# manycore-research/PlankAssembly

Measured on AMD Instinct MI355X. Metric: train samples/sec (fwd+bwd+all-reduce+Adam), d_model=512 seq=1024 [value: bf16 MFMA, f32 accumulate / master weights; train.f32 / train.x3: the same step in exact f32 / f32 with bf16x3 products = the parity paths], higher is better.
Workload: dtype bf16; 1 GPU; train_complete.yaml model d_model=512 H=8 dff=1024 6+6 post-norm layers, dropout 0.2, S=1024 (MAX_INPUT_LENGTH 1025), T=128, batch 16/GPU; global_batch=16, seq_len=1024, parallelism=dp1

## Files before the change

include/plank_hip.h:

```cpp
#ifndef PLANK_HIP_H
#define PLANK_HIP_H
#include <stdint.h>

#ifdef __cplusplus
extern "C" {
#endif

#define PA_F32 0
#define PA_BF16 1

#define PA_EINVAL (-1)
#define PA_EALIGN (-2)
#define PA_ESHAPE (-3)

int pa_version(void);

typedef struct {
    const void* A; const void* B; void* C;
    const float* bias;
    const void* R;
    const void* aux;
    void* ws;
    int32_t M, N, K;
    int32_t lda, ldb, ldc, ldr, ldaux;
// ... 216 lines not shown
                 float b2, float eps, int32_t step, float gscale, void* stream);
int pa_cast(void* dst, int32_t dst_dtype, const void* src, int32_t src_dtype, int64_t n, void* stream);

#define PA_GRAD_GUARD_PARTIALS 2048
typedef struct {
    float norm, coef, step_size, inv_sqrt_bc2;
    int32_t apply, applied, skipped, attempts, first_skipped_attempt;
    int32_t pad_[7];
} pa_grad_guard_ctl;
int64_t pa_grad_guard_ws_bytes(void);
int pa_grad_guard_init(void* ws, int64_t ws_bytes, int32_t step0, void* stream);
int pa_grad_guard(const float* g, int64_t n, float gscale, float max_norm, int32_t skip_nonfinite, float lr, float b1,
                  float b2, void* ws, int64_t ws_bytes, void* stream);
int pa_adam_step_guarded(float* p, const float* g, float* m, float* v, void* p_bf16, int64_t n, float b1, float b2,
                         float eps, float gscale, float clip_value, const pa_grad_guard_ctl* ctl, void* stream);
int pa_fake_collective(void* buf, int64_t bytes, int32_t blocks, int32_t passes, float min_us, void* stream);

typedef struct pa_model pa_model;
typedef struct {
    int32_t d_model, n_head, d_ff, n_enc, n_dec, vocab;
    int32_t out_dof;
    int32_t in_table_rows[5];
    float eps_layer, eps_final;
    int32_t has_enc_norm;
    float dropout;
    int32_t pad, end;
    int32_t dtype;
    int32_t activation;
} pa_model_cfg;
typedef struct {
// ... 18 lines not shown
int pa_model_create(const pa_model_cfg* cfg, pa_model** out);
void pa_model_destroy(pa_model* m);
int pa_model_num_params(const pa_model* m);
int pa_model_bind(pa_model* m, void* const* params_f32, void* const* params_lp, void* const* grads);
int pa_model_bind_transposed(pa_model* m, void* const* params_lpT);
int pa_model_bind_cross_kv_t(pa_model* m, const void* kvT_all);
int64_t pa_model_train_ws_bytes(pa_model* m, int32_t B, int32_t S, int32_t T);
#define PA_MODEL_STATS_FLOATS 8
int32_t pa_model_stats_floats(void);
int pa_model_train_fwd(pa_model* m, const pa_batch* batch, void* ws, int64_t ws_bytes, uint32_t seed,
                       int32_t training, float* stats, void* stream);
int pa_model_set_upstream(pa_model* m, const float* upstream);
int pa_model_train_num_segments(const pa_model* m);
int pa_model_train_bwd(pa_model* m, int32_t seg_lo, int32_t seg_hi, float gscale, void* stream);
int pa_model_grad_lag(const pa_model* m);
int pa_model_tensor(pa_model* m, int32_t which, void** ptr, int64_t* numel);

int64_t pa_decode_ws_bytes(pa_model* m, int32_t B, int32_t S, int32_t Tmax);
int pa_decode_begin(pa_model* m, void* ws, int64_t ws_bytes, int32_t Tmax, void* stream);
int pa_decode_step(pa_model* m, void* stream);
int pa_decode_step_pair(pa_model* a, pa_model* b, void* stream_a, void* stream_b);
int pa_decode_buffers(pa_model* m, void** tokens, void** attach, void** first_end, void** t_dev);
#define PA_BEAM_MAX 16
int64_t pa_decode_beam_ws_bytes(pa_model* m, int32_t rows, int32_t S, int32_t Tmax, int32_t K);
int pa_decode_beam_begin(pa_model* m, int32_t K, void* ws, int64_t ws_bytes, void* stream);
int pa_decode_beam_buffers(pa_model* m, void** scores, void** parents, void** finished);
typedef struct {
    uint32_t seed;
    int32_t n_per_drawing;
    float temperature;
// ... 52 lines not shown
```

plankassembly_amd/_lib.py:

```python
from __future__ import annotations

import ctypes as C
import os

import torch

HERE = os.path.dirname(os.path.abspath(__file__))
LIB_PATH = os.environ.get("PLANK_HIP_LIB") or os.path.join(HERE, "libplank_hip.so")

PA_F32, PA_BF16 = 0, 1
_ERR = {-1: "PA_EINVAL (bad argument)", -2: "PA_EALIGN (misaligned pointer / leading dimension)",
        -3: "PA_ESHAPE (unsupported shape)", -4: "PA_ESTATE (bad model/workspace state)"}


class PlankHipError(RuntimeError):
    pass


class GemmArgs(C.Structure):
    _fields_ = [("A", C.c_void_p), ("B", C.c_void_p), ("C", C.c_void_p), ("bias", C.c_void_p),
                ("R", C.c_void_p), ("aux", C.c_void_p), ("ws", C.c_void_p),
                ("M", C.c_int32), ("N", C.c_int32), ("K", C.c_int32),
                ("lda", C.c_int32), ("ldb", C.c_int32), ("ldc", C.c_int32), ("ldr", C.c_int32),
                ("ldaux", C.c_int32),
# ... 47 lines not shown
class AttnPlanInfo(C.Structure):
    _fields_ = [("n_launches", C.c_int32), ("balanced", C.c_int32), ("ks_min", C.c_int32), ("parts_q", C.c_int32),
                ("parts_kv", C.c_int32), ("sp_slots", C.c_int32), ("launch", AttnPlanLaunch * 3)]


class GroupDesc(C.Structure):
    _fields_ = [("idx", C.c_void_p), ("rowmap", C.c_void_p),
                ("n", C.c_int32), ("rows", C.c_int32), ("kind", C.c_int32), ("T", C.c_int32), ("dof", C.c_int32),
                ("tok_ld", C.c_int32), ("order", C.c_void_p), ("seg", C.c_void_p)]


class GradGuardCtl(C.Structure):
    _fields_ = [("norm", C.c_float), ("coef", C.c_float), ("step_size", C.c_float), ("inv_sqrt_bc2", C.c_float),
                ("apply", C.c_int32), ("applied", C.c_int32), ("skipped", C.c_int32), ("attempts", C.c_int32),
                ("first_skipped_attempt", C.c_int32), ("pad_", C.c_int32 * 7)]


GRAD_GUARD_PARTIALS = 2048
GRAD_GUARD_CTL_OFFSET = 4 * GRAD_GUARD_PARTIALS
GRAD_GUARD_WS_BYTES = GRAD_GUARD_CTL_OFFSET + C.sizeof(GradGuardCtl)

_lib = None


def _check_single_hip_runtime():
    try:
        maps = open("/proc/self/maps").read()
    except OSError:
        return
    libs = {ln.split()[-1] for ln in maps.splitlines() if "libamdhip64" in ln}
# ... 72 lines not shown
            "pa_attn_split_taken": (I64, [I]),
            "pa_gelu_fwd": (I, [P, P, I64, I, I, I, F, C.c_uint32, P]),
            "pa_gelu_bwd": (I, [P, P, P, I64, I, I, I, F, C.c_uint32, P]),
            "pa_switch_fwd": (I, [P, P, I, P, P, I64, I, P]),
            "pa_switch_bwd": (I, [P, I, P, P, P, P, I, P, P, I64, I, P]),
            "pa_mixture_nll_fwd": (I, [P, P, P, I, P, P, P, I, I, I, I, P]),
            "pa_mixture_nll_bwd": (I, [P, P, I, P, P, P, P, I, P, P, P, I, I, I, I, F, P]),
            "pa_mixture_nll_fwd_fin": (I, [P, P, P, I, P, P, P, I, I, I, I, P]),
            "pa_mixture_nll_bwd_up": (I, [P, P, I, P, P, P, P, I, P, P, P, I, I, I, I, F, P, P]),
            "pa_model_set_upstream": (I, [P, P]),
            "pa_adam_step": (I, [P, P, P, P, P, I64, F, F, F, F, I, F, P]),
            "pa_grad_guard_ws_bytes": (I64, []),
            "pa_grad_guard_init": (I, [P, I64, I, P]),
            "pa_grad_guard": (I, [P, I64, F, F, I, F, F, F, P, I64, P]),
            "pa_adam_step_guarded": (I, [P, P, P, P, P, I64, F, F, F, F, F, P, P]),
            "pa_cast": (I, [P, I, P, I, I64, P]),
            "pa_fake_collective": (I, [P, I64, I, I, F, P]),
            "pa_model_create": (I, [P, P]),
            "pa_model_destroy": (None, [P]),
            "pa_model_num_params": (I, [P]),
            "pa_model_bind": (I, [P, P, P, P]),
            "pa_model_bind_transposed": (I, [P, P]),
            "pa_model_bind_cross_kv_t": (I, [P, P]),
            "pa_transpose_many": (I, [P, I, I, I, P]),
            "pa_model_train_ws_bytes": (I64, [P, I, I, I]),
            "pa_model_train_fwd": (I, [P, P, P, I64, U, I, P, P]),
            "pa_model_train_num_segments": (I, [P]),
            "pa_model_stats_floats": (I, []),
            "pa_model_train_bwd": (I, [P, I, I, F, P]),
            "pa_model_grad_lag": (I, [P]),
            "pa_model_tensor": (I, [P, I, P, P]),
            "pa_decode_ws_bytes": (I64, [P, I, I, I]),
            "pa_decode_begin": (I, [P, P, I64, I, P]),
            "pa_decode_step": (I, [P, P]),
            "pa_decode_step_pair": (I, [P, P, P, P]),
            "pa_decode_buffers": (I, [P, P, P, P, P]),
            "pa_decode_beam_ws_bytes": (I64, [P, I, I, I, I]),
            "pa_decode_beam_begin": (I, [P, I, P, I64, P]),
            "pa_decode_beam_buffers": (I, [P, P, P, P]),
            "pa_decode_sample_ws_bytes": (I64, [P, I]),
            "pa_decode_sample_begin": (I, [P, P, P, I64, P]),
            "pa_decode_sample_set": (I, [P, P, P]),
            "pa_decode_sample_buffers": (I, [P, P]),
            "pa_decode_prefix_ws_bytes": (I64, [P, I, I]),
            "pa_decode_prefix_begin": (I, [P, P, P, P, P, I64, P]),
# ... 56 lines not shown
```

plankassembly_amd/csrc/rowops.hip:

```cpp
#include <type_traits>
#include "pa_device.h"
#include "../../include/plank_hip.h"

namespace {

constexpr int MAXV = 8;

struct EmbTabs { const float* t[5]; const int64_t* idx[5]; int n; const int32_t* rowmap; };
struct EmbGrads { float* t[5]; const int64_t* idx[5]; int rows[5]; int n; const int32_t* rowmap; };

template <typename T>
__global__ __launch_bounds__(256) void embed_input_fwd_kernel(T* out, EmbTabs tb, int64_t n_tok, int d) {
    const int vec_per_row = d >> 2;
    const int64_t total = n_tok * vec_per_row;
    for (int64_t e = (int64_t)blockIdx.x * blockDim.x + threadIdx.x; e < total; e += (int64_t)gridDim.x * blockDim.x) {
        const int64_t tok = e / vec_per_row;
        const int c = (int)(e % vec_per_row) << 2;
        const int64_t st = tb.rowmap ? (int64_t)tb.rowmap[tok] : tok;
        f32x4 acc = {0.f, 0.f, 0.f, 0.f};
#pragma unroll
        for (int k = 0; k < 5; ++k) {
            if (k < tb.n && tb.idx[k]) {
                const int64_t r = tb.idx[k][st];
                acc += *reinterpret_cast<const f32x4*>(tb.t[k] + r * d + c);
// ... 874 lines not shown
            pp[j] -= step_size * mm[j] / __builtin_fmaf(sqrtf(vv[j]), inv_sqrt_bc2, eps);
        }
        *reinterpret_cast<f32x4*>(p + e * 4) = pp;
        *reinterpret_cast<f32x4*>(m + e * 4) = mm;
        *reinterpret_cast<f32x4*>(v + e * 4) = vv;
        if (pb) st4<bf16>(pb + e * 4, pp);
    }
    if (blockIdx.x == 0 && threadIdx.x < (n & 3)) {
        const int64_t e = (n4 << 2) + threadIdx.x;
        float gj = g[e] * gscale * coef;
        gj = gj > clip ? clip : (gj < -clip ? -clip : gj);
        const float mj = __builtin_fmaf(b1, m[e], omb1 * gj);
        const float vj = __builtin_fmaf(b2, v[e], (omb2 * gj) * gj);
        m[e] = mj; v[e] = vj;
        p[e] -= step_size * mj / __builtin_fmaf(sqrtf(vj), inv_sqrt_bc2, eps);
        if (pb) pb[e] = (bf16)p[e];
    }
}

template <typename TD, typename TS>
__global__ __launch_bounds__(256) void cast_kernel(TD* dst, const TS* src, int64_t n) {
    for (int64_t e = (int64_t)blockIdx.x * blockDim.x + threadIdx.x; e < n; e += (int64_t)gridDim.x * blockDim.x)
        st1<TD>(dst + e, ld1<TS>(src + e));
}

inline int grid_for(int64_t work_items, int per_block = 256, int cap = 4096) {
    int64_t b = (work_items + per_block - 1) / per_block;
    if (b < 1) b = 1;
    return (int)(b > cap ? cap : b);
}
// ... 465 lines not shown
              reinterpret_cast<pa_grad_guard_ctl*>(static_cast<char*>(ws) + GUARD_CTL_OFFSET));
    return 0;
}

extern "C" int pa_adam_step_guarded(float* p, const float* g, float* m, float* v, void* p_bf16, int64_t n, float b1, float b2,
                                    float eps, float gscale, float clip_value, const pa_grad_guard_ctl* ctl, void* stream) {
    if (!p || !g || !m || !v || !ctl || n <= 0 || !(clip_value >= 0.f)) return PA_EINVAL;
    if ((reinterpret_cast<uintptr_t>(p) | reinterpret_cast<uintptr_t>(g) | reinterpret_cast<uintptr_t>(m) |
         reinterpret_cast<uintptr_t>(v)) & 15) return PA_EALIGN;
    if (reinterpret_cast<uintptr_t>(ctl) & 3) return PA_EALIGN;
    PA_LAUNCH(adam_guarded_kernel, dim3(grid_for(n >> 2, 256, 2048)), dim3(256), 0, ST(stream), p, g, m, v, (bf16*)p_bf16, n,
              b1, b2, eps, gscale, clip_value > 0.f ? clip_value : __builtin_inff(), ctl);
    return 0;
}

extern "C" int pa_cast(void* dst, int32_t dst_dtype, const void* src, int32_t src_dtype, int64_t n, void* stream) {
    if (!dst || !src || n <= 0) return PA_EINVAL;
    const int grid = grid_for(n, 256, 2048);
    if (dst_dtype == PA_BF16 && src_dtype == PA_F32) PA_LAUNCH((cast_kernel<bf16, float>), dim3(grid), dim3(256), 0, ST(stream), (bf16*)dst, (const float*)src, n);
    else if (dst_dtype == PA_F32 && src_dtype == PA_BF16) PA_LAUNCH((cast_kernel<float, bf16>), dim3(grid), dim3(256), 0, ST(stream), (float*)dst, (const bf16*)src, n);
    else if (dst_dtype == PA_F32 && src_dtype == PA_F32) PA_LAUNCH((cast_kernel<float, float>), dim3(grid), dim3(256), 0, ST(stream), (float*)dst, (const float*)src, n);
    else return PA_EINVAL;
    return 0;
}

__global__ __launch_bounds__(256) void fake_collective_kernel(f32x4* buf, long long n4, int passes, long long min_ticks) {
    const long long t0 = wall_clock64();
    const long long per = (n4 + gridDim.x - 1) / gridDim.x;
    const long long lo = per * blockIdx.x, hi = lo + per < n4 ? lo + per : n4;
    int pass = 0;
// ... 15 lines not shown
```

plankassembly_amd/csrc/runtime.hip:

```cpp
#include <stdlib.h>
#include <hip/hip_runtime.h>
#include <math.h>
#include <new>
#include <string.h>
#include <vector>
#include "../../include/plank_hip.h"

#include "model.h"

namespace {

#define RC(x) do { int rc_ = (x); if (rc_) return rc_; } while (0)

struct Ctx {
    pa_model* m; void* st;
    int dt() const { return m->cfg.dtype; }
    bool gelu() const { return m->cfg.activation == 2; }
    int ffn1(const void* A, const void* W, const float* bias, void* hidden, int rows, float drop_p, uint32_t seed) const {
        const int d = m->cfg.d_model, ff = m->cfg.d_ff;
        if (!gelu()) return linear(A, d, W, bias, hidden, ff, rows, ff, d, 1, drop_p, seed);
        RC(linear(A, d, W, bias, hidden, ff, rows, ff, d, 0));
        return pa_gelu_fwd(hidden, hidden, rows, ff, ff, dt(), drop_p, seed, st);
    }

// ... 712 lines not shown
extern "C" int pa_model_train_num_segments(const pa_model* m) {
    return m ? m->cfg.n_dec + m->cfg.n_enc + 4 : PA_EINVAL;
}

extern "C" int pa_model_train_bwd(pa_model* m, int32_t seg_lo, int32_t seg_hi, float gscale, void* stream) {
    if (!m || !m->have_fwd) return PA_EINVAL;
    for (int i = 0; i < m->n_params; ++i) if (!m->gr[i]) return PA_EINVAL;
    const int nseg = m->cfg.n_dec + m->cfg.n_enc + 4;
    if (seg_lo < 0 || seg_hi > nseg || seg_lo > seg_hi) return PA_EINVAL;
    for (int s = seg_lo; s < seg_hi; ++s) RC(backward_segment(m, s, gscale, stream));
    if (seg_hi == nseg && m->side_on) { RC(join_side(m, 0, stream)); RC(join_side(m, 1, stream)); m->select_set(0); }
    return 0;
}
extern "C" int pa_model_grad_lag(const pa_model* m) { return (m && m->side_on) ? 2 : 0; }

extern "C" int pa_model_tensor(pa_model* m, int32_t which, void** ptr, int64_t* numel) {
    if (!m || !ptr || !numel || m->B == 0) return PA_EINVAL;
    const int64_t d = m->cfg.d_model;
    switch (which) {
        case PA_T_MEMORY: *ptr = m->cfg.has_enc_norm ? m->memory : m->X[m->cfg.n_enc]; *numel = (int64_t)m->NE * d; return 0;
        case PA_T_HIDDENS: *ptr = m->hid; *numel = (int64_t)m->B * m->T * d; return 0;
        case PA_T_VOCAB_LOGITS: *ptr = m->vlog; *numel = (int64_t)m->B * m->T * m->ldv; return 0;
        case PA_T_PTR_LOGITS: *ptr = m->plog; *numel = (int64_t)m->B * m->T * m->T; return 0;
        default: break;
    }
    if (which >= PA_T_ENC_FFN(0) && which < PA_T_ENC_FFN(m->cfg.n_enc) && (int)m->ea.size() == m->cfg.n_enc) {
        *ptr = m->ea[which - PA_T_ENC_FFN(0)].hff; *numel = (int64_t)m->NE * m->cfg.d_ff; return *ptr ? 0 : PA_EINVAL;
    }
    if (which >= PA_T_DEC_FFN(0) && which < PA_T_DEC_FFN(m->cfg.n_dec) && (int)m->da.size() == m->cfg.n_dec) {
        *ptr = m->da[which - PA_T_DEC_FFN(0)].hff; *numel = (int64_t)m->B * m->T * m->cfg.d_ff; return *ptr ? 0 : PA_EINVAL;
// ... 4 lines not shown
```

plankassembly_amd/models.py:

```python
from __future__ import annotations

import ctypes as C
import math
import os
from collections import OrderedDict

import torch
import torch.nn as nn

from . import _lib as L


class _ModelCfg(C.Structure):
    _fields_ = [("d_model", C.c_int32), ("n_head", C.c_int32), ("d_ff", C.c_int32), ("n_enc", C.c_int32),
                ("n_dec", C.c_int32), ("vocab", C.c_int32), ("out_dof", C.c_int32), ("in_table_rows", C.c_int32 * 5),
                ("eps_layer", C.c_float), ("eps_final", C.c_float), ("has_enc_norm", C.c_int32),
                ("dropout", C.c_float), ("pad", C.c_int32), ("end", C.c_int32), ("dtype", C.c_int32),
                ("activation", C.c_int32)]


class _TrDesc(C.Structure):
    _fields_ = [("src", C.c_void_p), ("dst", C.c_void_p), ("rows", C.c_int32), ("cols", C.c_int32),
                ("ld_src", C.c_int32), ("ld_dst", C.c_int32), ("tile_begin", C.c_int32), ("pad_", C.c_int32)]

# ... 27 lines not shown
        keys += [p + "self_attn.in_proj_weight", p + "self_attn.in_proj_bias", p + "self_attn.out_proj.weight",
                 p + "self_attn.out_proj.bias", p + "linear1.weight", p + "linear1.bias", p + "linear2.weight",
                 p + "linear2.bias", p + "norm1.weight", p + "norm1.bias", p + "norm2.weight", p + "norm2.bias"]
    keys += ["encoder.norm.weight", "encoder.norm.bias"]
    for i in range(n_dec):
        p = f"decoder.layers.{i}."
        keys += [p + "self_attn.in_proj_weight", p + "self_attn.in_proj_bias", p + "self_attn.out_proj.weight",
                 p + "self_attn.out_proj.bias", p + "multihead_attn.in_proj_weight", p + "multihead_attn.in_proj_bias",
                 p + "multihead_attn.out_proj.weight", p + "multihead_attn.out_proj.bias", p + "linear1.weight",
                 p + "linear1.bias", p + "linear2.weight", p + "linear2.bias", p + "norm1.weight", p + "norm1.bias",
                 p + "norm2.weight", p + "norm2.bias", p + "norm3.weight", p + "norm3.bias"]
    keys += ["decoder.norm.weight", "decoder.norm.bias"]
    keys += ["vocab_head.weight", "vocab_head.bias", "pointer_head.weight", "pointer_head.bias",
             "switch_head.weight", "switch_head.bias"]
    return keys


class _Holder(nn.Module):

    def forward(self, *a, **k):
        raise RuntimeError("parameter container; the fused HIP path does the arithmetic")


def _xavier_(t):
    if t.dim() > 1:
        nn.init.xavier_uniform_(t)


class _TrainStepFn(torch.autograd.Function):

# ... 119 lines not shown
            n = math.prod(s)
            view = flat[self._offsets[k]: self._offsets[k] + n].view(s)
            prm = nn.Parameter(view)
            mod.register_parameter(parts[-1], prm)
            self._params[k] = prm
        if not self.has_enc_norm:
            del self.encoder._modules["norm"]
            for k in ("encoder.norm.weight", "encoder.norm.bias"):
                self._params[k].requires_grad_(False)
        self._flat = flat
        self._gflat = None
        self._gtmp = None
        self._shadow = None
        self._shadowT = self._vocabT = self._kvT = None
        self._tr_descs = None
        self._tr_stream = self._tr_event = None
        self._tr_pending = False
        self._shadow_version = -1
        self._handle = None
        self._ws = None
        self._stats = None
        self._step_seed = 0
        self._grad_hook = None
        self._hook_leaf = None
        self._decoder = None
        self._reset_parameters()

    def _reset_parameters(self):
        with torch.no_grad():
            for k, p in self._params.items():
# ... 27 lines not shown
        need = any(p.data.untyped_storage().data_ptr() != self._flat.untyped_storage().data_ptr()
                   or p.device != self._flat.device or p.dtype != torch.float32 for p in self._params.values())
        if not need:
            return
        flat = torch.zeros(self._numel, dtype=torch.float32, device=dev)
        with torch.no_grad():
            for k, p in self._params.items():
                n = p.numel()
                view = flat[self._offsets[k]: self._offsets[k] + n].view(self._shapes[k])
                view.copy_(p.data.to(torch.float32))
                p.data = view
                p.grad = None
        self._flat = flat
        self._gflat = self._gtmp = self._shadow = self._shadowT = self._vocabT = self._kvT = None
        self._tr_descs = None
        self._shadow_version = -1
        self._tr_stream = self._tr_event = None
        self._tr_pending = False
        self._drop_handle()

    def _drop_handle(self):
        if self._handle is not None:
            L.lib().pa_model_destroy(self._handle)
            self._handle = None
        self._ws = None
        self._decoder = None
        self._mode_decoders = {}
        self._drop_x3_cache()

    def _drop_x3_cache(self):
# ... 201 lines not shown
            tiles += ((s[0] + 63) // 64) * ((s[1] + 63) // 64)
            descs.append(d)
        nd, dm = self.num_decoder_layers, self.num_model
        self._kvT = None
        if bf and nd > 0 and dm % 8 == 0 and os.environ.get("PLANK_CROSS_KV", "1") != "0":
            self._kvT = torch.zeros(dm * nd * 2 * dm, dtype=torch.bfloat16, device=dev)
            for li in range(nd):
                k = f"decoder.layers.{li}.multihead_attn.in_proj_weight"
                src = self._shadow.data_ptr() + (self._offsets[k] + dm * dm) * 2
                dst = self._kvT.data_ptr() + li * 2 * dm * 2
                descs.append(_TrDesc(src, dst, 2 * dm, dm, dm, nd * 2 * dm, tiles, 0))
                tiles += ((2 * dm + 63) // 64) * ((dm + 63) // 64)
        arr = (_TrDesc * len(descs))(*descs)
        host = torch.frombuffer(bytearray(bytes(arr)), dtype=torch.uint8)
        self._tr_descs = (host.to(dev), len(descs), tiles)
        L.check(L.lib().pa_model_bind_transposed(self._handle, tab), "pa_model_bind_transposed")
        L.check(L.lib().pa_model_bind_cross_kv_t(self._handle, L.ptr(self._kvT) if self._kvT is not None else None),
                "pa_model_bind_cross_kv_t")

    def refresh_transposed(self):
        if self._tr_descs is not None:
            d, n, tiles = self._tr_descs
            dt = L.PA_BF16 if self.compute_dtype == "bf16" else L.PA_F32
            if os.environ.get("PLANK_TRANSPOSE_STREAM", "0") == "1":
                if self._tr_stream is None:
                    self._tr_stream, self._tr_event = torch.cuda.Stream(device=self._flat.device), torch.cuda.Event()
                self._tr_stream.wait_stream(torch.cuda.current_stream())
                with torch.cuda.stream(self._tr_stream):
                    L.check(L.lib().pa_transpose_many(L.ptr(d), n, tiles, dt, L.stream()), "pa_transpose_many")
                    self._tr_event.record(self._tr_stream)
                self._tr_pending = True
            else:
                L.check(L.lib().pa_transpose_many(L.ptr(d), n, tiles, dt, L.stream()), "pa_transpose_many")
        cache = getattr(self, "_x3_cache", None)
        if cache is not None:
            self.wait_transposed()
# ... 14 lines not shown
        return v

    def invalidate_shadow(self):
        self._shadow_version = -1

    def _refresh_shadow(self):
        v = self._param_version()
        if v != self._shadow_version:
            self.wait_transposed()
            if self.compute_dtype == "bf16":
                L.check(L.lib().pa_cast(L.ptr(self._shadow), L.PA_BF16, L.ptr(self._flat), L.PA_F32,
                                        C.c_int64(self._numel), L.stream()), "pa_cast")
            self._shadow_version = v
            self.refresh_transposed()

    def mark_shadow_fresh(self):
        self._shadow_version = self._param_version()
        self.refresh_transposed()

    def _make_batch(self, batch, with_output=True):
        iv = batch["input_value"]
        B, S = iv.shape
        keep = []
        b = _Batch()
        for i, k in enumerate(INPUT_KEYS):
            t = batch.get(k)
            if t is None:
                b.input_idx[i] = None
                continue
            t = t.to(device=self._flat.device, dtype=torch.int64).contiguous()
            keep.append(t)
            b.input_idx[i] = t.data_ptr()
        m = batch["input_mask"].to(self._flat.device).contiguous()
# ... 128 lines not shown
        if self._hook_leaf is None or self._hook_leaf.device != stats.device:
            self._hook_leaf = torch.zeros((), device=stats.device, requires_grad=True)
        if torch.is_grad_enabled():
            loss = _TrainStepFn.apply(self._hook_leaf, self, stats)
        else:
            loss = stats[4]
        return {"loss": loss, "accuracy": stats[5]}

    def _run_backward(self, gloss):
        self._ensure_grads()
        self.wait_transposed()
        accumulate = any(p.grad is not None for p in self._params.values())
        target = self._gflat
        if accumulate:
            if self._gtmp is None:
                self._gtmp = torch.empty_like(self._gflat)
            target = self._gtmp
        target.zero_()
        if self._bound_grads is not target:
            self._rebind(target)
        nseg = int(L.lib().pa_model_train_num_segments(self._handle))
        up = gloss if (gloss.dtype == torch.float32 and gloss.is_cuda and gloss.numel() == 1) else \
            gloss.reshape(1).to(device=self._flat.device, dtype=torch.float32)
        if not up.is_contiguous():
            up = up.contiguous()
        self._upstream_keep = up
        L.check(L.lib().pa_model_set_upstream(self._handle, L.ptr(up)), "pa_model_set_upstream")
        slices = self.segment_slices()
        hook = self._grad_hook
        self._sync_target = target
        lag = int(L.lib().pa_model_grad_lag(self._handle))
        for s in range(nseg):
            self._split(True, retain=True)
            try:
                L.check(L.lib().pa_model_train_bwd(self._handle, s, s + 1, C.c_float(1.0), L.stream()),
# ... 181 lines not shown
```

plankassembly_amd/optim.py:

```python
from __future__ import annotations

import ctypes as C
import math

import torch

from . import _lib as L


def _threshold(name, value):
    if value is None:
        return None
    if isinstance(value, bool) or not isinstance(value, (int, float)) or not math.isfinite(value) or value <= 0:
        raise ValueError(f"{name} must be a finite number above 0 (or None for off), got {value!r}")
    return float(value)


class FusedAdam(torch.optim.Optimizer):
    def __init__(self, model, lr=1e-4, betas=(0.9, 0.999), eps=1e-8, grad_scale=1.0, max_grad_norm=None, clip_value=None,
                 skip_nonfinite=False):
        max_grad_norm, clip_value = _threshold("max_grad_norm", max_grad_norm), _threshold("clip_value", clip_value)
        if max_grad_norm is not None and clip_value is not None:
            raise ValueError("max_grad_norm and clip_value are two clipping algorithms: set one of them")
        params = [p for p in model.parameters() if p.requires_grad]
# ... 13 lines not shown
            p.grad = None

    @torch.no_grad()
    def step(self, closure=None):
        loss = None
        if closure is not None:
            with torch.enable_grad():
                loss = closure()
        m = self.model
        flat, g = m.flat_params, m.flat_grads
        if self._m is None or self._m.device != flat.device:
            self._m = torch.zeros_like(flat)
            self._v = torch.zeros_like(flat)
        grp = self.param_groups[0]
        shadow = m._shadow if m.compute_dtype == "bf16" else None
        if self.guarded:
            self._guarded_step(flat, g, grp, shadow)
        else:
            self._plain_step(flat, g, grp, shadow)
        if shadow is not None:
            m.mark_shadow_fresh()
        else:
            m.invalidate_shadow()
        return loss

    def _plain_step(self, flat, g, grp, shadow):
        self._step += 1
        self.model.wait_transposed()
        L.check(L.lib().pa_adam_step(L.ptr(flat), L.ptr(g), L.ptr(self._m), L.ptr(self._v), L.ptr(shadow),
                                     C.c_int64(flat.numel()), C.c_float(grp["lr"]), C.c_float(grp["betas"][0]),
                                     C.c_float(grp["betas"][1]), C.c_float(grp["eps"]), self._step,
                                     C.c_float(self.grad_scale), L.stream()), "pa_adam_step")

    def _guarded_step(self, flat, g, grp, shadow):
        lib = L.lib()
        if self._ws is None or self._ws.device != flat.device:
            self._ws = torch.empty(L.GRAD_GUARD_WS_BYTES, dtype=torch.uint8, device=flat.device)
            self._ws_stale = True
        nws = C.c_int64(self._ws.numel())
        if self._ws_stale:
            L.check(lib.pa_grad_guard_init(L.ptr(self._ws), nws, int(self._step), L.stream()), "pa_grad_guard_init")
            self._ws_stale = False
        self._step += 1
        b1, b2 = grp["betas"]
        L.check(lib.pa_grad_guard(L.ptr(g), C.c_int64(g.numel()), C.c_float(self.grad_scale),
                                  C.c_float(self.max_grad_norm or 0.0), int(self.skip_nonfinite), C.c_float(grp["lr"]),
                                  C.c_float(b1), C.c_float(b2), L.ptr(self._ws), nws, L.stream()), "pa_grad_guard")
        self.model.wait_transposed()
        L.check(lib.pa_adam_step_guarded(L.ptr(flat), L.ptr(g), L.ptr(self._m), L.ptr(self._v), L.ptr(shadow),
                                         C.c_int64(flat.numel()), C.c_float(b1), C.c_float(b2), C.c_float(grp["eps"]),
                                         C.c_float(self.grad_scale), C.c_float(self.clip_value or 0.0),
                                         C.c_void_p(self._ws.data_ptr() + L.GRAD_GUARD_CTL_OFFSET), L.stream()),
                "pa_adam_step_guarded")

    def _ctl(self):
        if not self.guarded or self._ws is None or self._ws_stale:
            return None
        raw = self._ws[L.GRAD_GUARD_CTL_OFFSET:L.GRAD_GUARD_WS_BYTES].cpu().numpy().tobytes()
        return L.GradGuardCtl.from_buffer_copy(raw)

    def _applied_steps(self):
        c = self._ctl()
        return self._step if c is None else int(c.applied)
# ... 65 lines not shown
```

Measured before the change: 3475 samples/s.

## Fuse Adam update with transposed weight refresh and skip zeroing overwritten grads

Adds a tiled Adam kernel that updates parameters and writes the transposed low-precision weight copies (and cross-attention KV transposes) through LDS in the same pass. This removes the separate transpose refresh kernel that re-read the parameters after every optimizer step. It also adds a grad-zero plan that clears only the gradient ranges not fully overwritten by weight-gradient GEMMs, instead of zeroing the whole flat gradient buffer. Both are on by default via PLANK_STEP_TAIL=3. The cost is descriptor-table lookups per tile and more complex bookkeeping that must stay consistent with the GEMM overwrite semantics.

```diff
diff --git a/include/plank_hip.h b/include/plank_hip.h
--- a/include/plank_hip.h
+++ b/include/plank_hip.h
@@ -254,6 +254,19 @@
                   float b2, void* ws, int64_t ws_bytes, void* stream);
 int pa_adam_step_guarded(float* p, const float* g, float* m, float* v, void* p_bf16, int64_t n, float b1, float b2,
                          float eps, float gscale, float clip_value, const pa_grad_guard_ctl* ctl, void* stream);
+
+typedef struct {
+    int64_t off, count;
+    void* dst; void* dst2;
+    int32_t rows, cols, ld_dst, ld_dst2, row2, unit_begin;
+} pa_adam_desc;
+int64_t pa_adam_plan(pa_adam_desc* descs_host, int32_t n_desc, int64_t n, int32_t tr_dtype);
+int pa_adam_step_tr(float* p, const float* g, float* m, float* v, void* p_bf16, int64_t n, float lr, float b1, float b2,
+                    float eps, int32_t step, float gscale, const pa_adam_desc* descs_dev, int32_t n_desc, int32_t total_units,
+                    int32_t tr_dtype, void* stream);
+int pa_adam_step_tr_guarded(float* p, const float* g, float* m, float* v, void* p_bf16, int64_t n, float b1, float b2,
+                            float eps, float gscale, float clip_value, const pa_grad_guard_ctl* ctl,
+                            const pa_adam_desc* descs_dev, int32_t n_desc, int32_t total_units, int32_t tr_dtype, void* stream);
 int pa_fake_collective(void* buf, int64_t bytes, int32_t blocks, int32_t passes, float min_us, void* stream);
 
 typedef struct pa_model pa_model;
@@ -302,6 +315,8 @@
 int pa_model_train_num_segments(const pa_model* m);
 int pa_model_train_bwd(pa_model* m, int32_t seg_lo, int32_t seg_hi, float gscale, void* stream);
 int pa_model_grad_lag(const pa_model* m);
+int pa_model_grad_zero_plan(const pa_model* m, int64_t* offsets, int64_t* counts, int32_t cap);
+int pa_model_grad_zero(const pa_model* m, void* stream);
 int pa_model_tensor(pa_model* m, int32_t which, void** ptr, int64_t* numel);
 
 int64_t pa_decode_ws_bytes(pa_model* m, int32_t B, int32_t S, int32_t Tmax);
diff --git a/plankassembly_amd/_lib.py b/plankassembly_amd/_lib.py
--- a/plankassembly_amd/_lib.py
+++ b/plankassembly_amd/_lib.py
@@ -85,6 +85,12 @@
     _fields_ = [("norm", C.c_float), ("coef", C.c_float), ("step_size", C.c_float), ("inv_sqrt_bc2", C.c_float),
                 ("apply", C.c_int32), ("applied", C.c_int32), ("skipped", C.c_int32), ("attempts", C.c_int32),
                 ("first_skipped_attempt", C.c_int32), ("pad_", C.c_int32 * 7)]
+
+
+class AdamDesc(C.Structure):
+    _fields_ = [("off", C.c_int64), ("count", C.c_int64), ("dst", C.c_void_p), ("dst2", C.c_void_p),
+                ("rows", C.c_int32), ("cols", C.c_int32), ("ld_dst", C.c_int32), ("ld_dst2", C.c_int32),
+                ("row2", C.c_int32), ("unit_begin", C.c_int32)]
 
 
 GRAD_GUARD_PARTIALS = 2048
@@ -187,6 +193,9 @@
             "pa_grad_guard_init": (I, [P, I64, I, P]),
             "pa_grad_guard": (I, [P, I64, F, F, I, F, F, F, P, I64, P]),
             "pa_adam_step_guarded": (I, [P, P, P, P, P, I64, F, F, F, F, F, P, P]),
+            "pa_adam_plan": (I64, [P, I, I64, I]),
+            "pa_adam_step_tr": (I, [P, P, P, P, P, I64, F, F, F, F, I, F, P, I, I, I, P]),
+            "pa_adam_step_tr_guarded": (I, [P, P, P, P, P, I64, F, F, F, F, F, P, P, I, I, I, P]),
             "pa_cast": (I, [P, I, P, I, I64, P]),
             "pa_fake_collective": (I, [P, I64, I, I, F, P]),
             "pa_model_create": (I, [P, P]),
@@ -202,6 +211,8 @@
             "pa_model_stats_floats": (I, []),
             "pa_model_train_bwd": (I, [P, I, I, F, P]),
             "pa_model_grad_lag": (I, [P]),
+            "pa_model_grad_zero_plan": (I, [P, P, P, I]),
+            "pa_model_grad_zero": (I, [P, P]),
             "pa_model_tensor": (I, [P, I, P, P]),
             "pa_decode_ws_bytes": (I64, [P, I, I, I]),
             "pa_decode_begin": (I, [P, P, I64, I, P]),
diff --git a/plankassembly_amd/csrc/grad_zero_plan.h b/plankassembly_amd/csrc/grad_zero_plan.h
--- /dev/null
+++ b/plankassembly_amd/csrc/grad_zero_plan.h
@@ -0,0 +1,56 @@
+#pragma once
+#include "model.h"
+
+static inline int64_t pa_overwritten_weight_numel(const pa_model* m, int i) {
+    const pa_model_cfg& c = m->cfg;
+    const int64_t d = c.d_model, ff = c.d_ff;
+    if (i >= m->enc_base(0) && i < m->enc_norm()) {
+        switch ((i - m->enc_base(0)) % E_COUNT) {
+        case E_IN_W: return 3 * d * d;
+        case E_OUT_W: return d * d;
+        case E_L1_W: case E_L2_W: return d * ff;
+        default: return 0;
+        }
+    }
+    if (i >= m->dec_base(0) && i < m->dec_norm()) {
+        switch ((i - m->dec_base(0)) % D_COUNT) {
+        case D_SA_IN_W: case D_CA_IN_W: return 3 * d * d;
+        case D_SA_OUT_W: case D_CA_OUT_W: return d * d;
+        case D_L1_W: case D_L2_W: return d * ff;
+        default: return 0;
+        }
+    }
+    if (i == m->tail() + T_VOCAB_W) return (int64_t)c.vocab * d;
+    if (i == m->tail() + T_PTR_W) return d * d;
+    return 0;
+}
+
+static inline int pa_grad_zero_plan_impl(const pa_model* m, int64_t* offsets, int64_t* counts, int32_t cap) {
+    if (!m || cap < 0 || (cap > 0 && (!offsets || !counts))) return PA_EINVAL;
+    const int n = m->n_params;
+    for (int i = 0; i < n; ++i) if (!m->gr[i]) return PA_EINVAL;
+    const char* base = (const char*)m->gr[0];
+    if (reinterpret_cast<uintptr_t>(base) & 15) return PA_EALIGN;
+    const int64_t total = ((const char*)m->gr[n - 1] - base) / 4 + 1;
+    int ns = 0;
+    int64_t lo = 0;
+    auto emit = [&](int64_t hi) {
+        if (hi > lo) {
+            if (ns < cap) { offsets[ns] = lo; counts[ns] = hi - lo; }
+            ++ns;
+        }
+    };
+    for (int i = 0; i < n; ++i) {
+        const ptrdiff_t b = (const char*)m->gr[i] - base;
+        const ptrdiff_t next = i + 1 < n ? (const char*)m->gr[i + 1] - base : (ptrdiff_t)total * 4;
+        if (b < 0 || (b & 3) || next <= b) return PA_EINVAL;
+        const int64_t w = pa_overwritten_weight_numel(m, i);
+        if (w == 0) continue;
+        if ((b & 15) || (w & 3)) return PA_EALIGN;
+        if (b / 4 + w > next / 4) return PA_EINVAL;
+        emit(b / 4);
+        lo = b / 4 + w;
+    }
+    emit(total);
+    return ns;
+}
diff --git a/plankassembly_amd/csrc/rowops.hip b/plankassembly_amd/csrc/rowops.hip
--- a/plankassembly_amd/csrc/rowops.hip
+++ b/plankassembly_amd/csrc/rowops.hip
@@ -912,6 +912,111 @@
         const float vj = __builtin_fmaf(b2, v[e], (omb2 * gj) * gj);
         m[e] = mj; v[e] = vj;
         p[e] -= step_size * mj / __builtin_fmaf(sqrtf(vj), inv_sqrt_bc2, eps);
+        if (pb) pb[e] = (bf16)p[e];
+    }
+}
+
+constexpr int ADAM_TR = 64, ADAM_TC = 64, ADAM_FLAT = 4096;
+
+__device__ __forceinline__ f32x4 adam_ld(const float* p) { return *reinterpret_cast<const f32x4*>(p); }
+__device__ __forceinline__ void adam_st(float* p, f32x4 x) { *reinterpret_cast<f32x4*>(p) = x; }
+
+struct AdamK { float step_size, inv_sqrt_bc2, gs, coef, clip, b1, b2, omb1, omb2, eps; };
+
+template <bool GUARDED>
+__device__ __forceinline__ void adam_update4(f32x4& pp, const f32x4& gg, f32x4& mm, f32x4& vv, const AdamK& k) {
+#pragma unroll
+    for (int j = 0; j < 4; ++j) {
+        float gj = gg[j] * k.gs;
+        if (GUARDED) {
+            gj = gj * k.coef;
+            gj = gj > k.clip ? k.clip : (gj < -k.clip ? -k.clip : gj);
+        }
+        mm[j] = __builtin_fmaf(k.omb1, gj, k.b1 * mm[j]);
+        vv[j] = __builtin_fmaf(k.b2, vv[j], (k.omb2 * gj) * gj);
+        pp[j] -= k.step_size * mm[j] / __builtin_fmaf(sqrtf(vv[j]), k.inv_sqrt_bc2, k.eps);
+    }
+}
+
+template <typename TD, bool GUARDED>
+__global__ __launch_bounds__(256) __attribute__((amdgpu_waves_per_eu(4, 8))) void adam_tr_kernel(float* p, const float* g, float* m, float* v, bf16* pb, int64_t n,
+                                                      const pa_adam_desc* descs, int n_desc, int total_units, AdamK k,
+                                                      const pa_grad_guard_ctl* ctl) {
+    constexpr int G = 16 / (int)sizeof(TD);
+    constexpr int PITCH = ADAM_TR + G;
+    constexpr int TPR = ADAM_TC / 4, RPP = 256 / TPR, PASSES = ADAM_TR / RPP;
+    __shared__ __attribute__((aligned(16))) TD lds[ADAM_TC * PITCH];
+    if (GUARDED) {
+        if (ctl->apply == 0) return;
+        k.step_size = ctl->step_size; k.inv_sqrt_bc2 = ctl->inv_sqrt_bc2; k.coef = ctl->coef;
+    }
+    for (int u = blockIdx.x; u < total_units; u += gridDim.x) {
+        int lo = 0, hi = n_desc - 1;
+        while (lo < hi) {
+            const int mid = (lo + hi + 1) >> 1;
+            if (descs[mid].unit_begin <= u) lo = mid; else hi = mid - 1;
+        }
+        const pa_adam_desc d = descs[lo];
+        const int t = u - d.unit_begin;
+        if (d.dst == nullptr) {
+            const int64_t cnt4 = d.count >> 2;
+#pragma unroll
+            for (int i = 0; i < ADAM_FLAT / 1024; ++i) {
+                const int64_t e4 = (int64_t)t * (ADAM_FLAT / 4) + i * 256 + threadIdx.x;
+                if (e4 >= cnt4) break;
+                const int64_t e = d.off + e4 * 4;
+                f32x4 pp = adam_ld(p + e), gg = adam_ld(g + e), mm = adam_ld(m + e), vv = adam_ld(v + e);
+                adam_update4<GUARDED>(pp, gg, mm, vv, k);
+                adam_st(p + e, pp); adam_st(m + e, mm); adam_st(v + e, vv);
+                if (pb) st4<bf16>(pb + e, pp);
+            }
+            continue;
+        }
+        const int tiles_c = (d.cols + ADAM_TC - 1) / ADAM_TC;
+        const int r0 = (t / tiles_c) * ADAM_TR, c0 = (t % tiles_c) * ADAM_TC;
+        const int tr = threadIdx.x / TPR, tc = (threadIdx.x % TPR) * 4;
+#pragma unroll
+        for (int h = 0; h < PASSES; ++h) {
+            const int rl = tr + RPP * h;
+            if (r0 + rl >= d.rows || c0 + tc >= d.cols) continue;
+            const int64_t e = d.off + (int64_t)(r0 + rl) * d.cols + c0 + tc;
+            f32x4 pp = adam_ld(p + e), gg = adam_ld(g + e), mm = adam_ld(m + e), vv = adam_ld(v + e);
+            adam_update4<GUARDED>(pp, gg, mm, vv, k);
+            adam_st(p + e, pp); adam_st(m + e, mm); adam_st(v + e, vv);
+            if (pb) st4<bf16>(pb + e, pp);
+#pragma unroll
+            for (int j = 0; j < 4; ++j) lds[(tc + j) * PITCH + rl] = (TD)pp[j];
+        }
+        __syncthreads();
+        constexpr int TPD = ADAM_TR / G;
+        for (int i = threadIdx.x; i < ADAM_TC * TPD; i += 256) {
+            const int cl = i / TPD, rg = (i % TPD) * G;
+            const int c = c0 + cl, r = r0 + rg;
+            if (c >= d.cols || r >= d.rows) continue;
+            const TD* s = lds + cl * PITCH + rg;
+            TD* o = reinterpret_cast<TD*>(d.dst) + (int64_t)c * d.ld_dst + r;
+            if (r + G <= d.rows) {
+                *reinterpret_cast<u32x4*>(o) = *reinterpret_cast<const u32x4*>(s);
+                if (d.dst2 && r >= d.row2)
+                    *reinterpret_cast<u32x4*>(reinterpret_cast<TD*>(d.dst2) + (int64_t)c * d.ld_dst2 + (r - d.row2)) =
+                        *reinterpret_cast<const u32x4*>(s);
+            } else {
+                for (int j = 0; r + j < d.rows; ++j) o[j] = s[j];
+            }
+        }
+        __syncthreads();
+    }
+    if (blockIdx.x == 0 && threadIdx.x < (n & 3)) {
+        const int64_t e = ((n >> 2) << 2) + threadIdx.x;
+        float gj = g[e] * k.gs;
+        if (GUARDED) {
+            gj = gj * k.coef;
+            gj = gj > k.clip ? k.clip : (gj < -k.clip ? -k.clip : gj);
+        }
+        const float mj = __builtin_fmaf(k.b1, m[e], k.omb1 * gj);
+        const float vj = __builtin_fmaf(k.b2, v[e], (k.omb2 * gj) * gj);
+        m[e] = mj; v[e] = vj;
+        p[e] -= k.step_size * mj / __builtin_fmaf(sqrtf(vj), k.inv_sqrt_bc2, k.eps);
         if (pb) pb[e] = (bf16)p[e];
     }
 }
@@ -1407,6 +1512,86 @@
     return 0;
 }
 
+extern "C" int64_t pa_adam_plan(pa_adam_desc* descs, int32_t n_desc, int64_t n, int32_t tr_dtype) {
+    if (!descs || n_desc <= 0 || n <= 0 || (tr_dtype != PA_BF16 && tr_dtype != PA_F32)) return PA_EINVAL;
+    const int G = tr_dtype == PA_BF16 ? 8 : 4;
+    int64_t end = 0, units = 0;
+    for (int i = 0; i < n_desc; ++i) {
+        pa_adam_desc& d = descs[i];
+        if (d.off != end || d.count <= 0 || d.count > n - d.off) return PA_EINVAL;
+        if (d.off & 3) return PA_EALIGN;
+        end = d.off + d.count;
+        if ((d.count & 3) && end != n) return PA_EALIGN;
+        if (units > 0x7fffffff) return PA_EINVAL;
+        d.unit_begin = (int32_t)units;
+        if (!d.dst) {
+            if (d.dst2) return PA_EINVAL;
+            units += ((d.count >> 2 << 2) + ADAM_FLAT - 1) / ADAM_FLAT;
+            continue;
+        }
+        if (d.rows <= 0 || d.cols <= 0 || (int64_t)d.rows * d.cols != d.count || d.ld_dst < d.rows) return PA_EINVAL;
+        if ((d.cols & 3) || d.ld_dst % G || (reinterpret_cast<uintptr_t>(d.dst) & 15)) return PA_EALIGN;
+        if (d.dst2) {
+            if (d.row2 < 0 || d.row2 >= d.rows || d.ld_dst2 < d.rows - d.row2) return PA_EINVAL;
+            if (d.rows % G || d.row2 % G || d.ld_dst2 % G || (reinterpret_cast<uintptr_t>(d.dst2) & 15)) return PA_EALIGN;
+        }
+        units += (int64_t)((d.rows + ADAM_TR - 1) / ADAM_TR) * ((d.cols + ADAM_TC - 1) / ADAM_TC);
+    }
+    if (end != n || units > 0x7fffffff) return PA_EINVAL;
+    return units;
+}
+
+static int adam_tr_args_check(const float* p, const float* g, const float* m, const float* v, const void* p_bf16, int64_t n,
+                              const pa_adam_desc* descs_dev, int32_t n_desc, int32_t total_units, int32_t tr_dtype) {
+    if (!p || !g || !m || !v || n <= 0 || !descs_dev || n_desc <= 0 || total_units < 0) return PA_EINVAL;
+    if (tr_dtype == PA_BF16 ? !p_bf16 : (tr_dtype != PA_F32 || p_bf16)) return PA_EINVAL;
+    if ((reinterpret_cast<uintptr_t>(p) | reinterpret_cast<uintptr_t>(g) | reinterpret_cast<uintptr_t>(m) |
+         reinterpret_cast<uintptr_t>(v)) & 15) return PA_EALIGN;
+    if (reinterpret_cast<uintptr_t>(p_bf16) & 7) return PA_EALIGN;
+    return 0;
+}
+
+extern "C" int pa_adam_step_tr(float* p, const float* g, float* m, float* v, void* p_bf16, int64_t n, float lr, float b1,
+                               float b2, float eps, int32_t step, float gscale, const pa_adam_desc* descs_dev, int32_t n_desc,
+                               int32_t total_units, int32_t tr_dtype, void* stream) {
+    if (int rc = adam_tr_args_check(p, g, m, v, p_bf16, n, descs_dev, n_desc, total_units, tr_dtype)) return rc;
+    if (step < 1) return PA_EINVAL;
+    const double bc1 = 1.0 - pow((double)b1, (double)step), bc2 = 1.0 - pow((double)b2, (double)step);
+    AdamK k;
+    k.step_size = (float)((double)lr / bc1); k.inv_sqrt_bc2 = (float)(1.0 / sqrt(bc2));
+    k.gs = gscale; k.coef = 1.f; k.clip = __builtin_inff();
+    k.b1 = b1; k.b2 = b2; k.omb1 = 1.f - b1; k.omb2 = 1.f - b2; k.eps = eps;
+    const dim3 grid(total_units > 0 ? total_units : 1);
+    if (tr_dtype == PA_BF16)
+        PA_LAUNCH((adam_tr_kernel<bf16, false>), grid, dim3(256), 0, ST(stream), p, g, m, v, (bf16*)p_bf16, n, descs_dev, n_desc,
+                  total_units, k, (const pa_grad_guard_ctl*)nullptr);
+    else
+        PA_LAUNCH((adam_tr_kernel<float, false>), grid, dim3(256), 0, ST(stream), p, g, m, v, (bf16*)nullptr, n, descs_dev, n_desc,
+                  total_units, k, (const pa_grad_guard_ctl*)nullptr);
+    return 0;
+}
+
+extern "C" int pa_adam_step_tr_guarded(float* p, const float* g, float* m, float* v, void* p_bf16, int64_t n, float b1, float b2,
+                                       float eps, float gscale, float clip_value, const pa_grad_guard_ctl* ctl,
+                                       const pa_adam_desc* descs_dev, int32_t n_desc, int32_t total_units, int32_t tr_dtype,
+                                       void* stream) {
+    if (int rc = adam_tr_args_check(p, g, m, v, p_bf16, n, descs_dev, n_desc, total_units, tr_dtype)) return rc;
+    if (!ctl || !(clip_value >= 0.f)) return PA_EINVAL;
+    if (reinterpret_cast<uintptr_t>(ctl) & 3) return PA_EALIGN;
+    AdamK k;
+    k.step_size = 0.f; k.inv_sqrt_bc2 = 0.f; k.coef = 1.f;
+    k.gs = gscale; k.clip = clip_value > 0.f ? clip_value : __builtin_inff();
+    k.b1 = b1; k.b2 = b2; k.omb1 = 1.f - b1; k.omb2 = 1.f - b2; k.eps = eps;
+    const dim3 grid(total_units > 0 ? total_units : 1);
+    if (tr_dtype == PA_BF16)
+        PA_LAUNCH((adam_tr_kernel<bf16, true>), grid, dim3(256), 0, ST(stream), p, g, m, v, (bf16*)p_bf16, n, descs_dev, n_desc,
+                  total_units, k, ctl);
+    else
+        PA_LAUNCH((adam_tr_kernel<float, true>), grid, dim3(256), 0, ST(stream), p, g, m, v, (bf16*)nullptr, n, descs_dev, n_desc,
+                  total_units, k, ctl);
+    return 0;
+}
+
 extern "C" int pa_cast(void* dst, int32_t dst_dtype, const void* src, int32_t src_dtype, int64_t n, void* stream) {
     if (!dst || !src || n <= 0) return PA_EINVAL;
     const int grid = grid_for(n, 256, 2048);
diff --git a/plankassembly_amd/csrc/runtime.hip b/plankassembly_amd/csrc/runtime.hip
--- a/plankassembly_amd/csrc/runtime.hip
+++ b/plankassembly_amd/csrc/runtime.hip
@@ -7,6 +7,8 @@
 #include "../../include/plank_hip.h"
 
 #include "model.h"
+#include "grad_zero_plan.h"
+#include "pa_device.h"
 
 namespace {
 
@@ -750,6 +752,59 @@
 }
 extern "C" int pa_model_grad_lag(const pa_model* m) { return (m && m->side_on) ? 2 : 0; }
 
+namespace {
+
+constexpr int GZ_SLICES = 96;
+constexpr int GZ_CHUNK = 1024;
+struct GradZeroTab {
+    int n;
+    int chunk_begin[GZ_SLICES + 1];
+    int64_t off[GZ_SLICES];
+    int64_t cnt[GZ_SLICES];
+};
+
+__global__ __launch_bounds__(256) void grad_zero_kernel(float* base, GradZeroTab t) {
+    int s = 0;
+    while (s + 1 < t.n && (int)blockIdx.x >= t.chunk_begin[s + 1]) ++s;
+    const int64_t e = (int64_t)((int)blockIdx.x - t.chunk_begin[s]) * GZ_CHUNK + (int64_t)threadIdx.x * 4;
+    const int64_t cnt = t.cnt[s];
+    float* p = base + t.off[s] + e;
+    if (e + 4 <= cnt) {
+        *reinterpret_cast<float4*>(p) = make_float4(0.f, 0.f, 0.f, 0.f);
+    } else {
+        for (int j = 0; e + j < cnt; ++j) p[j] = 0.f;
+    }
+}
+
+}
+
+extern "C" int pa_model_grad_zero_plan(const pa_model* m, int64_t* offsets, int64_t* counts, int32_t cap) {
+    return pa_grad_zero_plan_impl(m, offsets, counts, cap);
+}
+
+extern "C" int pa_model_grad_zero(const pa_model* m, void* stream) {
+    int ns = pa_model_grad_zero_plan(m, nullptr, nullptr, 0);
+    if (ns < 0) return ns;
+    std::vector<int64_t> o(ns), c(ns);
+    ns = pa_model_grad_zero_plan(m, o.data(), c.data(), ns);
+    if (ns < 0) return ns;
+    for (int s0 = 0; s0 < ns; s0 += GZ_SLICES) {
+        GradZeroTab t;
+        t.n = ns - s0 < GZ_SLICES ? ns - s0 : GZ_SLICES;
+        t.chunk_begin[0] = 0;
+        for (int s = 0; s < GZ_SLICES; ++s) {
+            const bool live = s < t.n;
+            t.off[s] = live ? o[s0 + s] : 0; t.cnt[s] = live ? c[s0 + s] : 0;
+            const int64_t chunks = (t.cnt[s] + GZ_CHUNK - 1) / GZ_CHUNK;
+            if (chunks > 0x7fffffff - t.chunk_begin[s]) return PA_EINVAL;
+            t.chunk_begin[s + 1] = t.chunk_begin[s] + (int)chunks;
+        }
+        if (t.chunk_begin[t.n] == 0) continue;
+        PA_LAUNCH(grad_zero_kernel, dim3(t.chunk_begin[t.n]), dim3(256), 0, (hipStream_t)stream, (float*)m->gr[0], t);
+    }
+    return 0;
+}
+
 extern "C" int pa_model_tensor(pa_model* m, int32_t which, void** ptr, int64_t* numel) {
     if (!m || !ptr || !numel || m->B == 0) return PA_EINVAL;
     const int64_t d = m->cfg.d_model;
diff --git a/plankassembly_amd/models.py b/plankassembly_amd/models.py
--- a/plankassembly_amd/models.py
+++ b/plankassembly_amd/models.py
@@ -65,6 +65,10 @@
     keys += ["vocab_head.weight", "vocab_head.bias", "pointer_head.weight", "pointer_head.bias",
              "switch_head.weight", "switch_head.bias"]
     return keys
+
+
+def _step_tail():
+    return int(os.environ.get("PLANK_STEP_TAIL", "3"))
 
 
 class _Holder(nn.Module):
@@ -214,6 +218,7 @@
         self._shadow = None
         self._shadowT = self._vocabT = self._kvT = None
         self._tr_descs = None
+        self._adam_descs = None
         self._tr_stream = self._tr_event = None
         self._tr_pending = False
         self._shadow_version = -1
@@ -271,6 +276,7 @@
         self._flat = flat
         self._gflat = self._gtmp = self._shadow = self._shadowT = self._vocabT = self._kvT = None
         self._tr_descs = None
+        self._adam_descs = None
         self._shadow_version = -1
         self._tr_stream = self._tr_event = None
         self._tr_pending = False
@@ -502,12 +508,44 @@
         arr = (_TrDesc * len(descs))(*descs)
         host = torch.frombuffer(bytearray(bytes(arr)), dtype=torch.uint8)
         self._tr_descs = (host.to(dev), len(descs), tiles)
+        self._adam_descs = self._adam_table(tab, dev) if _step_tail() & 1 else None
         L.check(L.lib().pa_model_bind_transposed(self._handle, tab), "pa_model_bind_transposed")
         L.check(L.lib().pa_model_bind_cross_kv_t(self._handle, L.ptr(self._kvT) if self._kvT is not None else None),
                 "pa_model_bind_cross_kv_t")
 
-    def refresh_transposed(self):
-        if self._tr_descs is not None:
+    def _adam_table(self, tab, dev):
+        bf = self.compute_dtype == "bf16"
+        esz = 2 if bf else 4
+        nd, dm = self.num_decoder_layers, self.num_model
+        descs, end = [], 0
+
+        def flat_to(off):
+            if off > end:
+                descs.append(L.AdamDesc(end, off - end, None, None, 0, 0, 0, 0, 0, 0))
+
+        for i, k in enumerate(self._order):
+            if not tab[i]:
+                continue
+            s, off = self._shapes[k], self._offsets[k]
+            flat_to(off)
+            ld = (s[0] + 63) // 64 * 64 if k == "vocab_head.weight" else s[0]
+            dst2, ld2, row2 = None, 0, 0
+            if self._kvT is not None and k.startswith("decoder.layers.") and k.endswith("multihead_attn.in_proj_weight"):
+                li = int(k.split(".")[2])
+                dst2, ld2, row2 = self._kvT.data_ptr() + li * 2 * dm * esz, nd * 2 * dm, dm
+            descs.append(L.AdamDesc(off, s[0] * s[1], tab[i], dst2, s[0], s[1], ld, ld2, row2, 0))
+            end = off + s[0] * s[1]
+        flat_to(self._numel)
+        arr = (L.AdamDesc * len(descs))(*descs)
+        dt = L.PA_BF16 if bf else L.PA_F32
+        units = int(L.lib().pa_adam_plan(arr, len(descs), C.c_int64(self._numel), dt))
+        if units < 0:
+            L.check(units, "pa_adam_plan")
+        host = torch.frombuffer(bytearray(bytes(arr)), dtype=torch.uint8)
+        return host.to(dev), len(descs), units, dt
+
+    def refresh_transposed(self, fresh=False):
+        if self._tr_descs is not None and not fresh:
             d, n, tiles = self._tr_descs
             dt = L.PA_BF16 if self.compute_dtype == "bf16" else L.PA_F32
             if os.environ.get("PLANK_TRANSPOSE_STREAM", "0") == "1":
@@ -552,9 +590,14 @@
             self._shadow_version = v
             self.refresh_transposed()
 
-    def mark_shadow_fresh(self):
+    def mark_shadow_fresh(self, transposed=False):
         self._shadow_version = self._param_version()
-        self.refresh_transposed()
+        self.refresh_transposed(fresh=transposed)
+
+    def adam_table(self):
+        if self._tr_descs is None or os.environ.get("PLANK_TRANSPOSE_STREAM", "0") == "1":
+            return None
+        return self._adam_descs
 
     def _make_batch(self, batch, with_output=True):
         iv = batch["input_value"]
@@ -713,11 +756,14 @@
         target = self._gflat
         if accumulate:
             if self._gtmp is None:
-                self._gtmp = torch.empty_like(self._gflat)
+                self._gtmp = torch.zeros_like(self._gflat)
             target = self._gtmp
-        target.zero_()
         if self._bound_grads is not target:
             self._rebind(target)
+        if _step_tail() & 2:
+            L.check(L.lib().pa_model_grad_zero(self._handle, L.stream()), "pa_model_grad_zero")
+        else:
+            target.zero_()
         nseg = int(L.lib().pa_model_train_num_segments(self._handle))
         up = gloss if (gloss.dtype == torch.float32 and gloss.is_cuda and gloss.numel() == 1) else \
             gloss.reshape(1).to(device=self._flat.device, dtype=torch.float32)
diff --git a/plankassembly_amd/optim.py b/plankassembly_amd/optim.py
--- a/plankassembly_amd/optim.py
+++ b/plankassembly_amd/optim.py
@@ -51,25 +51,34 @@
             self._v = torch.zeros_like(flat)
         grp = self.param_groups[0]
         shadow = m._shadow if m.compute_dtype == "bf16" else None
+        table = m.adam_table()
         if self.guarded:
-            self._guarded_step(flat, g, grp, shadow)
+            self._guarded_step(flat, g, grp, shadow, table)
         else:
-            self._plain_step(flat, g, grp, shadow)
-        if shadow is not None:
-            m.mark_shadow_fresh()
+            self._plain_step(flat, g, grp, shadow, table)
+        if shadow is not None or table is not None:
+            m.mark_shadow_fresh(transposed=table is not None)
         else:
             m.invalidate_shadow()
         return loss
 
-    def _plain_step(self, flat, g, grp, shadow):
+    def _plain_step(self, flat, g, grp, shadow, table=None):
         self._step += 1
         self.model.wait_transposed()
+        if table is not None:
+            descs, n_desc, units, dt = table
+            L.check(L.lib().pa_adam_step_tr(L.ptr(flat), L.ptr(g), L.ptr(self._m), L.ptr(self._v), L.ptr(shadow),
+                                            C.c_int64(flat.numel()), C.c_float(grp["lr"]), C.c_float(grp["betas"][0]),
+                                            C.c_float(grp["betas"][1]), C.c_float(grp["eps"]), self._step,
+                                            C.c_float(self.grad_scale), L.ptr(descs), n_desc, units, dt, L.stream()),
+                    "pa_adam_step_tr")
+            return
         L.check(L.lib().pa_adam_step(L.ptr(flat), L.ptr(g), L.ptr(self._m), L.ptr(self._v), L.ptr(shadow),
                                      C.c_int64(flat.numel()), C.c_float(grp["lr"]), C.c_float(grp["betas"][0]),
                                      C.c_float(grp["betas"][1]), C.c_float(grp["eps"]), self._step,
                                      C.c_float(self.grad_scale), L.stream()), "pa_adam_step")
 
-    def _guarded_step(self, flat, g, grp, shadow):
+    def _guarded_step(self, flat, g, grp, shadow, table=None):
         lib = L.lib()
         if self._ws is None or self._ws.device != flat.device:
             self._ws = torch.empty(L.GRAD_GUARD_WS_BYTES, dtype=torch.uint8, device=flat.device)
@@ -84,6 +93,14 @@
                                   C.c_float(self.max_grad_norm or 0.0), int(self.skip_nonfinite), C.c_float(grp["lr"]),
                                   C.c_float(b1), C.c_float(b2), L.ptr(self._ws), nws, L.stream()), "pa_grad_guard")
         self.model.wait_transposed()
+        if table is not None:
+            descs, n_desc, units, dt = table
+            L.check(lib.pa_adam_step_tr_guarded(L.ptr(flat), L.ptr(g), L.ptr(self._m), L.ptr(self._v), L.ptr(shadow),
+                                                C.c_int64(flat.numel()), C.c_float(b1), C.c_float(b2), C.c_float(grp["eps"]),
+                                                C.c_float(self.grad_scale), C.c_float(self.clip_value or 0.0),
+                                                C.c_void_p(self._ws.data_ptr() + L.GRAD_GUARD_CTL_OFFSET), L.ptr(descs),
+                                                n_desc, units, dt, L.stream()), "pa_adam_step_tr_guarded")
+            return
         L.check(lib.pa_adam_step_guarded(L.ptr(flat), L.ptr(g), L.ptr(self._m), L.ptr(self._v), L.ptr(shadow),
                                          C.c_int64(flat.numel()), C.c_float(b1), C.c_float(b2), C.c_float(grp["eps"]),
                                          C.c_float(self.grad_scale), C.c_float(self.clip_value or 0.0),
```

New measurement: 3509 samples/s (median of 6 runs). Within noise of the previous version (+1.0%).
